# jenndrei/BayHunter

Hardware: AMD Instinct MI355X
Metric: forward-model+logL evals/sec (batched 10-layer models) (higher is better)
Workload: dtype f64

## Files before the change

### bayhunter_amd/csrc/bh_device.h

```cpp
#pragma once
#include <hip/hip_runtime.h>
#include <stddef.h>
#include <stdint.h>

#define BH_WAVE 64
#define BH_COUNTER_WORDS 16
#define BH_TRACE_WAVES 16384
#define BH_DEBUG_WORDS (BH_COUNTER_WORDS + 4 * BH_TRACE_WAVES)
#define BH_BOARD_WORDS (2 * 32768)

__device__ __forceinline__ double bh_rcp_refined(double b)
{
    double r = __builtin_amdgcn_rcp(b);
    double e = __builtin_fma(-b, r, 1.0);
    r = __builtin_fma(r, e, r);
    e = __builtin_fma(-b, r, 1.0);
    r = __builtin_fma(r, e, r);
    return r;
}
__device__ __forceinline__ double bh_quot(double a, double b, double r)
{
    const double q = a * r;
    const double rem = __builtin_fma(-b, q, a);
    return __builtin_fma(rem, r, q);
// ... 72 lines not shown
    int Lcut;
    int rows[2], lanes[2];
    int wg_n0, wg_n1;
    unsigned long long *neval;
    unsigned *board;
    unsigned stamp;
    unsigned *started;
    int prio_low;
    int fast;
    int adapt_ok;
    int counted;
    int rerun;
    int farith;
    int restart;
    SwdTarget t[8];
};
struct SwdSiteXArgs {
    const int32_t *site;
    int nsites, nt, ldx;
    const int32_t *n;
    const double *x;
    int col[8], off[8];
};
__device__ __forceinline__ int bh_site_count(const SwdSiteXArgs &X, int ty, int ib, int cap)
{
    const int s = X.site[ib];
    if (s < 0 || s >= X.nsites) return -1;
    const int n = X.n[(size_t)s * X.nt + X.col[ty]];
    return n < 0 ? 0 : (n > cap ? cap : n);
}
// ... 8 lines not shown
double bh_swd_plan(int B, int Lmax, int ntargets, const int *iwave, int Gforce, int *G, int *look);
size_t bh_swd_group_lds_bytes(int G, int J, int Lmax, int Kmax, int maxmode, bool sitex = false);
struct SwdPairWork {
    int ncu = 0;
    int32_t *perm[2] = {nullptr, nullptr};
    int32_t *slot_rank[2] = {nullptr, nullptr};
    int cap_perm = 0, cap_rank[2] = {0, 0};
    int key_n0 = -1, key_n1 = -1;
};
struct PairOrderTarget {
    int mpw, nwaves;
    const int32_t *slot_rank;
    int32_t *perm;
    int xcd;
};
bool bh_pair_order_fits(int B);
void bh_launch_pair_order(int B, int Lmax, const int32_t *nlay, const double *vs, ptrdiff_t sl, ptrdiff_t sb, int nt,
                          const PairOrderTarget *tg, hipStream_t stream);
struct SwdLaunchInfo {
    unsigned workgroups;
    long waves;
    size_t lds;
    int wpb;
};
inline int bh_trials_fit(int G, int look)
{
    int J = look > 1 ? look : 1;
    while (J > 1 && G * J > BH_WAVE) --J;
    return J;
}
struct SwdGroupAsk {
// ... 174 lines not shown
```

### bayhunter_amd/csrc/bh_engine.hip

```cpp
#include "../../include/bh_engine_debug.h"
#include "../../include/bh_engine_sites.h"
#include "../../include/bh_engine_sites_rf.h"
#include "../../include/bh_engine_sites_x.h"
#include "../../include/bh_engine_sites_x_all.h"
#include "../../include/bh_engine_sites_missing.h"
#include "../../include/bh_engine_sites_gauss.h"
#include "../../include/bh_engine_sites_rf_axis.h"
#include "bh_device.h"

#include <algorithm>
#include <cmath>
#include <cstdio>
#include <cstdlib>
#include <cstring>
#include <new>
#include <string>
#include <vector>

#include "bh_tuning.h"
#include <cstring>
#include <mutex>

namespace {
BhTuning g_tuning;
// ... 121 lines not shown
    DevBuf gc_xn;
    DevBuf gc_work;
    bool timing = false, counting = false;
    bool no_mfma = false;
    bool as_given = false;
    int force_group = 0;
    int force_look = 0;
    int hint_layers = 0;
    int swd_search = BH_SEARCH_FAST;
    int swd_arith = BH_ARITH_FAST;
    int swd_scan = 2;
    DevBuf guard;
    uint64_t rerun_launches = 0;
    uint64_t guard_total[BH_MAX_TARGETS] = {0};
    bool guard_fresh = true;
    bool guard_last = false;
    struct EventSet {
        hipEvent_t ev[8];
        bool used[4];
    };
    std::vector<EventSet> evsets;
    size_t ncalls = 0;
    uint64_t last_neval = 0;
    bool neval_pending = false;
};

namespace {

int fail(bh_engine *e, int code, const char *what, hipError_t he = hipSuccess)
{
// ... 195 lines not shown
int swd_counter(bh_engine *e, hipStream_t st, unsigned long long **out)
{
    *out = nullptr;
    if (!e->counting) return BH_OK;
    int rc = ensure(e, e->counter, BH_DEBUG_WORDS * sizeof(unsigned long long));
    if (rc) return rc;
    if (!e->neval_pending) {
        HIPCHK(e, hipMemsetAsync(e->counter.p, 0, BH_COUNTER_WORDS * sizeof(unsigned long long), st));
        e->neval_pending = true;
    }
    *out = (unsigned long long *)e->counter.p;
    return BH_OK;
}

constexpr int GUARD_HEAD = 24;
int guard_space(bh_engine *e, hipStream_t st, int B, int32_t **counts, int32_t **lists)
{
    const size_t need = ((size_t)GUARD_HEAD + (size_t)BH_MAX_TARGETS * (size_t)(B + 4)) * sizeof(int32_t);
    if (need > e->guard.cap) {
        if (e->guard.p) {
            int32_t cum[BH_MAX_TARGETS];
            HIPCHK(e, hipStreamSynchronize(st));
            HIPCHK(e, hipMemcpy(cum, (int32_t *)e->guard.p + 2 * BH_MAX_TARGETS, sizeof(cum), hipMemcpyDeviceToHost));
            for (int t = 0; t < BH_MAX_TARGETS; ++t) e->guard_total[t] += (uint64_t)(uint32_t)cum[t];
        }
        e->guard_fresh = true;
    }
    int rc = ensure(e, e->guard, need);
    if (rc) return rc;
    *counts = (int32_t *)e->guard.p;
    *lists = (int32_t *)e->guard.p + GUARD_HEAD;
    HIPCHK(e, hipMemsetAsync(e->guard.p, 0, (e->guard_fresh ? GUARD_HEAD : 2 * BH_MAX_TARGETS) * sizeof(int32_t), st));
    e->guard_fresh = false;
    return BH_OK;
}

bool takes_fast(int search, const SwdJob &J)
{
    return J.igr == BH_VEL_PHASE && J.mode <= 1 && (search == BH_SEARCH_FAST || (search == BH_SEARCH_FAST_RAYLEIGH && J.iwave == BH_WAVE_RAYLEIGH));
}

enum SwdOrder { ORDER_NONE, ORDER_DEPTH, ORDER_LENGTH, ORDER_PAIR };

struct SwdPlan {
    bool first_roots[BH_MAX_TARGETS];
    int nsplit;
    int ntargets, kmax, maxmode;
    bool any_sphere;
    int typ_layers;
    int kernel;
    int G, lean_trials;
    int order, Lcut;
    int len_mpw, len_xcd;
    bool sitex;
    bool any_fast, farith, adapt_ok;
    int job[BH_MAX_TARGETS], look[BH_MAX_TARGETS], inlook[BH_MAX_TARGETS], look_group[BH_MAX_TARGETS];
    bool fast[BH_MAX_TARGETS], refseq[BH_MAX_TARGETS];
};

SwdPlan plan_swd(const bh_engine *e, int B, int Lmax, int typ_given, int njobs, const SwdJob *jobs)
{
    const BhTuning &tun = bh_tuning();
    SwdPlan p{};
    p.maxmode = 1;
    for (int j = 0; j < njobs; ++j) p.sitex = p.sitex || jobs[j].sx.tab != nullptr;
    int iw[BH_MAX_TARGETS], nfast = 0;
    for (int j = 0; j < njobs; ++j) {
        const SwdJob &J = jobs[j];
// ... 45 lines not shown
            wmax = w > wmax ? w : wmax;
        }
        const int pair_min = tun.swd_pair_minwaves;
        if (plan_waves >= (pair_min >= 0 ? pair_min : 7 * (long)e->pairwork.ncu) && (pair_min >= 0 || 2 * wmax >= 3 * wmin))
            p.order = ORDER_PAIR;
    }
    p.Lcut = Lmax;
    if (ordered && p.order != ORDER_PAIR) {
        if (lean && bh_pair_order_fits(B) && tun.swd_lean_no_sort == 0) {
            p.order = ORDER_LENGTH;
            p.len_mpw = 1;
            const int mpw = BH_WAVE / p.lean_trials, per_wg = (nlive == 2) ? 2 : 4;
            if (tun.swd_lean_xcd != 0 && tun.swd_lean_r < 4 && tun.swd_lean_l < 4 && B % mpw == 0 && B % 8 == 0 && (B / mpw) % (8 * per_wg) == 0) {
                p.len_mpw = mpw;
                p.len_xcd = per_wg;
            }
        } else {
            p.order = ORDER_DEPTH;
            if (shallow_bulk) p.Lcut = p.typ_layers + 2;
        }
    }
    p.any_fast = nfast > 0;
    p.farith = e->swd_arith == BH_ARITH_FAST;
    p.adapt_ok = e->force_group == 0 && e->force_look == 0 && tun.swd_look_r == 0 && tun.swd_look_l == 0;
    for (int t = 0; t < nlive; ++t) {
        p.refseq[t] = nfast > 0 && jobs[p.job[t]].igr == BH_VEL_PHASE && !p.fast[t];
        if (p.kernel == BH_KERNEL_LANE) {
            p.look[t] = look[t] > 1 ? look[t] : 1;
            continue;
        }
// ... 168 lines not shown
}

unsigned swd_stamp(bh_engine *e)
{
    const unsigned s = (++e->swd_stamp) & 0xffffu;
    return s != 0 ? s : (++e->swd_stamp) & 0xffffu;
}

int wait_for(bh_engine *e, hipEvent_t ev, hipStream_t from, hipStream_t to)
{
    HIPCHK(e, hipEventRecord(ev, from));
    HIPCHK(e, hipStreamWaitEvent(to, ev, 0));
    return BH_OK;
}

void note_launch(bh_engine *e, int family, int role, const int key[6], bool two, bool inter, bool pair, bool restart, unsigned grid_x, int fair)
{
    if (e->n_swd_launches >= (int)(sizeof(e->swd_launches) / sizeof(e->swd_launches[0]))) return;
    bh_swd_launch &r = e->swd_launches[e->n_swd_launches++];
    r.family = family; r.role = role;
    for (int k = 0; k < 6; ++k) r.key[k] = key[k];
    r.two_classes = two; r.interleaved = inter; r.pair_order = pair; r.restart = restart; r.grid_x = (int)grid_x; r.fair = fair;
}
void note_lane(bh_engine *e, int role, const SwdLaneBuild &b) { note_launch(e, BH_KERNEL_LANE, role, b.key, false, false, false, false, b.grid_x, b.fair); }
void note_group(bh_engine *e, int role, const SwdGroupPlan &g, bool pair)
{
    const SwdGroupBuild &b = g.build;
    const int key[6] = {b.fastm, b.simple, b.prof, b.adapt, b.cntb, b.fa};
    note_launch(e, BH_KERNEL_GROUP, role, key, g.grid.z == 2, g.wg_n1 > 0, pair, g.restart, g.grid.x, 0);
}

void set_group_args(SwdMultiArgs &a, const SwdGroupPlan &g)
{
    for (int k = 0; k < 2; ++k) {
        a.rows[k] = g.rows[k];
        a.lanes[k] = g.lanes[k];
    }
// ... 52 lines not shown
            target_of(W, ty, wid);
            if (ty == t && wid < nw[t] - 1) v.emplace_back(q[(size_t)W], wid);
        }
        std::sort(v.begin(), v.end());
        rank[t].assign((size_t)(nw[t] > 0 ? nw[t] : 1), 0);
        for (size_t r = 0; r < v.size(); ++r) rank[t][(size_t)v[r].second] = (int32_t)r;
    }
    return true;
}

int launch_swd_rerun(bh_engine *e, hipStream_t st, const SwdMultiArgs &main, int32_t *counts, int32_t *lists, const SwdSiteXArgs *sx = nullptr)
{
    SwdMultiArgs a = main;
    a.rerun = 1;
    a.perm = nullptr;
    a.split = nullptr;
    a.Lcut = a.Lmax;
    a.started = nullptr;
    a.stamp = swd_stamp(e);
    a.adapt_ok = 1;
    SwdGroupAsk q{};
    q.B = a.B; q.Lmax = q.Lcut = a.Lmax; q.ntargets = a.ntargets;
    q.G0 = bh_swd_pick_group(a.B, a.ntargets, a.Lmax);
    for (int t = 0; t < a.ntargets; ++t) {
        SwdTarget &T = a.t[t];
        T.perm = lists + (size_t)t * (size_t)(a.B + 4);
        T.count = counts + t;
        T.gcount = nullptr;
        T.glist = nullptr;
        T.look = 64 / q.G0 > 1 ? 64 / q.G0 : 1;
// ... 50 lines not shown
        PairOrderTarget tg[2];
        for (int t = 0; t < nt; ++t) tg[t] = PairOrderTarget{g.pair_mpw[t], n[t], geom ? pw.slot_rank[t] : nullptr, pw.perm[t]};
        const SwdTarget t0 = swd_target(c, c.p.job[0]);
        bh_launch_pair_order(B, c.Lmax, c.m.nlay, t0.vs, t0.sl, t0.sb, nt, tg, c.st);
        for (int t = 0; t < nt; ++t) c.pair_perm[t] = pw.perm[t];
    }
    (void)hipGetLastError();
    return BH_OK;
}

int order_models(SwdCall &c)
{
    const SwdPlan &p = c.p;
    if (p.order == ORDER_NONE) return BH_OK;
    if (p.order == ORDER_PAIR) return c.g.pair ? pair_models(c) : BH_OK;
    bh_engine *e = c.e;
    int rc;
    if ((rc = ensure(e, e->perm, ((size_t)c.B + 4) * sizeof(int32_t)))) return rc;
    int32_t *perm = (int32_t *)e->perm.p;
    if (p.order == ORDER_LENGTH) {
        const PairOrderTarget tg{p.len_mpw, c.B / p.len_mpw, nullptr, perm + 4, p.len_xcd};
        bh_launch_pair_order(c.B, c.Lmax, c.m.nlay, c.m.vs, c.sl, c.sb, 1, &tg, c.st);
    } else {
        bh_launch_order(c.B, c.m.nlay, perm + 4, p.Lcut, perm, c.st);
        c.split = (p.Lcut < c.Lmax) ? perm : nullptr;
    }
    c.perm = perm + 4;
    return BH_OK;
}

// ... 35 lines not shown
    if (fork && (rc = wait_for(e, e->ev_join2, e->aux2, c.st))) return rc;
    HIPCHK(e, hipGetLastError());
    return BH_OK;
}

int launch_swd_multi(SwdCall &c, SwdMultiArgs &a)
{
    bh_engine *e = c.e;
    const SwdPlan &p = c.p;
    const int B = c.B;
    int rc;
    if ((rc = swd_board(e, c.st, &a.board))) return rc;
    a.stamp = swd_stamp(e);
    a.B = B; a.Lmax = c.Lmax; a.nlay = c.m.nlay; a.neval = c.counter; a.perm = c.perm;
    a.split = c.split; a.Lcut = p.Lcut;
    a.ntargets = p.ntargets;
    for (int t = 0; t < p.ntargets; ++t) {
        a.t[t] = swd_target(c, p.job[t]);
        a.t[t].look = p.look[t];
        a.t[t].inlook = p.inlook[t];
        a.t[t].refseq = p.refseq[t] ? 1 : 0;
    }
    a.started = e->started;
    a.prio_low = c.prio_low;
    a.adapt_ok = p.adapt_ok ? 1 : 0;
    if (p.sitex) {
        c.sx = *c.jobs[p.job[0]].sx.tab;
        for (int t = 0; t < p.ntargets; ++t) {
            c.sx.col[t] = c.jobs[p.job[t]].sx.col;
            c.sx.off[t] = c.jobs[p.job[t]].sx.off;
// ... 5 lines not shown
        a.farith = p.farith ? 1 : 0;
        a.fast = p.any_fast ? 1 : 0;
    } else {
        for (int t = 0; t < 2; ++t) a.t[t].perm = c.pair_perm[t];
        set_group_args(a, c.g);
    }
    if (bh_tuning().debug_plan != 0) {
        std::fprintf(stderr, "[bh] dispersion plan B=%d Lmax=%d: lanes per model %d, typical layers %d (hint %d), Lcut %d%s, pairing %d; trials per round:",
                     B, c.Lmax, p.G, c.m.typ_layers, e->hint_layers, p.Lcut, p.Lcut < c.Lmax ? " (two depth classes)" : "", (int)(p.order == ORDER_PAIR));
        for (int t = 0; t < p.ntargets; ++t) std::fprintf(stderr, " %s %d/%d", a.t[t].iwave == BH_WAVE_LOVE ? "L" : "R", p.look_group[t], p.inlook[t]);
        if (!lean) std::fprintf(stderr, "; launched lanes per model %d/%d", c.g.lanes[0], c.g.lanes[1]);
        std::fprintf(stderr, "\n");
    }
    e->guard_last = p.any_fast;
    if (p.any_fast) {
        if ((rc = guard_space(e, c.st, B, &c.gcounts, &c.glists))) return rc;
        for (int t = 0; t < a.ntargets; ++t)
            if (a.t[t].igr == BH_VEL_PHASE) {
                a.t[t].gcount = c.gcounts + t;
                a.t[t].glist = c.glists + (size_t)t * (size_t)(B + 4);
            }
    }
    ev_begin(e, 0, c.st);
    e->last_swd_kernel = p.kernel;
    if (lean) {
        SwdLaneBuild lb{};
        if ((p.sitex ? bh_launch_swd_lean_x(a, c.sx, c.st, &c.info, &lb) : bh_launch_swd_lean(a, c.st, &c.info, &lb)) != 0)
            return fail(e, BH_EINVAL, "model too deep for LDS");
        note_launch(e, BH_KERNEL_LEAN, BH_SWD_MAIN, lb.key, false, p.ntargets == 2, false, false, lb.grid_x, 0);
    } else {
        if (!p.sitex) bh_launch_swd_group(a, c.g, c.st);
        else if (!bh_launch_swd_group_x(a, c.g, c.sx, c.st)) return fail(e, BH_EUNSUPPORTED, "no site-period build of this dispersion launch");
        note_group(e, BH_SWD_MAIN, c.g, c.pair_perm[0] != nullptr);
        c.info = c.g.info;
    }
    const hipError_t le = hipGetLastError();
    if (le != hipSuccess) return fail(e, BH_EHIP, "dispersion kernel launch", le);
    if (e->started) e->started_expected += c.info.workgroups;
    return BH_OK;
}

int launch_second_roots(const SwdCall &c)
{
    bh_engine *e = c.e;
    const int B = c.B;
    const bool sitex = c.p.sitex && e->site_x_all;
    int J2 = 16;
    {
        long searches = 0;
        for (int t = 0; t < c.p.ntargets; ++t) searches += c.p.first_roots[c.p.job[t]] ? (long)B * c.jobs[c.p.job[t]].K : 0;
        while (J2 > 1 && searches * J2 > 2048L * 64) J2 >>= 1;
    }
    size_t off[BH_MAX_TARGETS + 1] = {0};
// ... 273 lines not shown
}
int bh_engine_set_swd_trials(bh_engine *e, int trials)
{
    if (!e) return BH_EINVAL;
    if (trials != 0 && trials != 4 && trials != 8 && trials != 16 && trials != 32 && trials != 64)
        return fail(e, BH_EINVAL, "trials must be 0 (by the call's shape), 4, 8, 16, 32 or 64");
    e->swd_trials = trials;
    return BH_OK;
}
int bh_engine_get_swd_trials(const bh_engine *e) { return e ? e->swd_trials : 0; }
int bh_engine_guard_stats(bh_engine *e, int32_t *counts, uint64_t *rerun_launches, uint64_t *total)
{
    if (!e) return BH_EINVAL;
    if (rerun_launches) *rerun_launches = e->rerun_launches;
    if (counts || total) {
        int32_t w[3 * BH_MAX_TARGETS] = {0};
        if (e->guard.p && !e->guard_fresh) {
            HIPCHK(e, hipDeviceSynchronize());
            HIPCHK(e, hipMemcpy(w, e->guard.p, sizeof(w), hipMemcpyDeviceToHost));
        }
        if (counts)
            for (int t = 0; t < BH_MAX_TARGETS; ++t) counts[t] = e->guard_last ? w[t] + w[BH_MAX_TARGETS + t] : 0;
        if (total)
            for (int t = 0; t < BH_MAX_TARGETS; ++t) total[t] = e->guard_total[t] + (uint64_t)(uint32_t)w[2 * BH_MAX_TARGETS + t];
    }
    return BH_OK;
}

int bh_engine_set_swd_lookahead(bh_engine *e, int trials_per_round)
{
    if (!e) return BH_EINVAL;
    if (trials_per_round < 0 || trials_per_round > 16)
        return fail(e, BH_EINVAL, "look-ahead must be 0 (auto) or 1..16 trial velocities per round");
    e->force_look = trials_per_round;
    return BH_OK;
}

int bh_engine_set_swd_group(bh_engine *e, int lanes_per_model)
{
// ... 861 lines not shown
```

### bayhunter_amd/csrc/bh_tuning.h

```cpp
#pragma once

#define BH_TUNING_TABLE(X)                                                                                                          \
    X(swd_search,        "BH_SWD_SEARCH",        -1, "initial root refinement: r(eference) / f(ast) / fast_rayleigh; -1 = the library's default")    \
    X(swd_scan,          "BH_SWD_SCAN",          -1, "initial scan mode: s(teps) / c(ounted) / a(uto); -1 = auto")                                  \
    X(swd_arith,         "BH_SWD_ARITH",         -1, "initial arithmetic of short-refinement launches: e(xact) / f(ast); -1 = the library's default") \
    X(swd_group,         "BH_SWD_GROUP",          0, "lanes per model of the dispersion kernel (0 = planned per launch)")                           \
    X(swd_lookahead,     "BH_SWD_LOOKAHEAD",      0, "trial velocities per round (0 = planned per launch)")                                         \
    X(swd_look_r,        "BH_SWD_LOOK_R",         0, "trials per round of Rayleigh wavefronts only (0 = planned)")                                  \
    X(swd_look_l,        "BH_SWD_LOOK_L",         0, "trials per round of Love wavefronts only (0 = planned)")                                      \
    X(swd_love_inlook,   "BH_SWD_LOVE_INLOOK",    0, "Love trials inside a lane group, 1..4 (0 = automatic)")                                       \
    X(swd_prio_low,      "BH_SWD_PRIO_LOW",      -1, "issue priority of a dispersion wavefront's unfavoured phase beside RF wavefronts (-1 = 1)")    \
    X(swd_pair_minwaves, "BH_SWD_PAIR_MINWAVES", -1, "wavefronts from which the SIMD-pairing order of the models is used (-1 = 7 x CUs)")           \
    X(swd_slice,         "BH_SWD_SLICE",          0, "lane-per-model kernel: rounds between priority changes (0 = default)")                        \
    X(swd_hint_always,   "BH_SWD_HINT_ALWAYS",    0, "flag: honour the typical-depth hint also when every model gets a wavefront")                   \
    X(swd_no_pair,       "BH_SWD_NO_PAIR",        0, "flag: no SIMD-pairing order of the models")                                                    \
    X(swd_no_mix,        "BH_SWD_NO_MIX",         0, "flag: Rayleigh and Love wavefronts not interleaved in the grid")                               \
    X(swd_no_adapt,      "BH_SWD_NO_ADAPT",       0, "flag: one-model-per-wavefront launches do not size lane groups per model")                     \
    X(swd_no_restart,    "BH_SWD_NO_RESTART",     0, "flag: guarded models are re-run by a second launch instead of restarting in place")            \
    X(swd_no_simple,     "BH_SWD_NO_SIMPLE",      0, "flag: no kernel build specialised for fundamental-mode phase velocities")                      \
    X(swd_no_board,      "BH_SWD_NO_BOARD",       0, "flag: no progress board between the two wavefronts of a SIMD")                                 \
    X(swd_no_fair,       "BH_SWD_NO_FAIR",        0, "flag: no alternating issue priority of the two wavefronts of a SIMD")                          \
    X(swd_redundant,     "BH_SWD_REDUNDANT",      0, "flag: every lane of a group runs the whole Rayleigh recursion")                                \
    X(swd_no_lean,       "BH_SWD_NO_LEAN",        0, "flag: fast-arithmetic launches take the group / lane kernels' FA builds, not the trial-per-lane kernel") \
    X(swd_lean_pairs,    "BH_SWD_LEAN_PAIRS",     0, "trial-per-lane kernel: largest call in (model, target) pairs that takes it (0 = 2^20)")        \
    X(swd_lean_no_sort,  "BH_SWD_LEAN_NO_SORT",   0, "flag: trial-per-lane kernel: models by depth only, not by predicted search length")           \
    X(swd_lean_r,        "BH_SWD_LEAN_R",         0, "trial-per-lane kernel: trials per round of Rayleigh targets, power of two 4..64 (0 = planned)")  \
    X(swd_lean_l,        "BH_SWD_LEAN_L",         0, "trial-per-lane kernel: trials per round of Love targets (0 = planned)")                         \
    X(swd_lean_xcd,      "BH_SWD_LEAN_XCD",       1, "trial-per-lane kernel: 1 = the models ordered inside eight blocks of the batch, a block per XCD (0: one order for the chip)") \
    X(swd_rerun_wgs,     "BH_SWD_RERUN_WGS",    256, "workgroups per target of the re-run launch of guarded models, striding over the list (0 = one wavefront per model of the batch, as before round 6)") \
    X(swd_gsplit,        "BH_SWD_GSPLIT",  16777216, "group velocities (fundamental mode): calls of up to this many (model, period) pairs per target -- 2^24, the most the launch indexes -- run the chain of first roots and the second roots as two launches (0 = one search after the other in one launch)") \
    X(swd_lean_flip,     "BH_SWD_LEAN_FLIP",    256, "trial-per-lane kernel, two targets: 256 = the second target takes the models in the opposite order (0: the same order); + n: the targets of a wavefront pair swap with bit n-1 of the workgroup index") \
    X(no_order,          "BH_NO_ORDER",           0, "flag: models processed in the caller's order")                                                 \
    X(no_overlap,        "BH_NO_OVERLAP",         0, "flag: receiver function after the dispersion kernel, not beside it")                           \
    X(no_started,        "BH_NO_STARTED",         0, "flag: no start gate (stream memory operation) for the receiver-function stream")               \
    X(no_mfma,           "BH_NO_MFMA",            0, "flag: Gauss-law quadratic form in like_kernel instead of the MFMA contraction")                \
    X(err_memset,        "BH_ERR_MEMSET",         0, "flag: zero the per-target failure flags on every call")                                        \
    X(gauss_tile,        "BH_GAUSS_TILE",         0, "tile of the Gauss-law contraction: 64 / 128 (0 = automatic)")                                  \
    X(rf_lds_beside,     "BH_RF_LDS_BESIDE",     -1, "LDS floor (bytes) of receiver-function workgroups beside an ungated dispersion launch (-1 = default)") \
    X(rf_lds_gated,      "BH_RF_LDS_GATED",       0, "LDS floor (bytes) of receiver-function workgroups of a gated fused call (0 = none)")           \
    X(rf_keep_floor,     "BH_RF_KEEP_FLOOR",      0, "flag: keep the ungated LDS floor in a gated fused call")                                       \
    X(rf_coef_big,       "BH_RF_COEF_BIG",        0, "flag: the large-register coefficient kernel also beside the dispersion kernel")                \
    X(rf_no_fuse,        "BH_RF_NO_FUSE",         0, "flag: the receiver function always writes its trace (no fused likelihood)")                    \
    X(rf_no_cut,         "BH_RF_NO_CUT",          0, "flag: every frequency bin computed (no spectral cut-off below 1e-17)")                         \
// ... 17 lines not shown
```

### bayhunter_amd/csrc/swd_kernel.hip

```cpp
#include "../../include/bh_engine_debug.h"
#include "bh_device.h"
#include "bh_tuning.h"
#include <cmath>
#include <cstdlib>

#define BH_HD __device__ __forceinline__
#define BH_TAB static __device__ const
#include "bh_libm.h"

namespace {
#include "swd_common.h"

constexpr int LANE_TAB_PAD = (LIBM_TAB_BYTES + 15) & ~15;
#ifndef BH_NEV_LO
#define BH_NEV_LO 5
#endif
constexpr int NEV_LO = BH_NEV_LO;
__host__ __device__ inline size_t lane_wave_bytes(int Lmax, int K, int mode)
{
    const size_t b = (size_t)4 * Lmax * 64 * sizeof(float) + (size_t)2 * NEV_LO * 64 * sizeof(double) +
                     (size_t)((K + 1) & ~1) * sizeof(double) + (mode > 1 ? (size_t)2 * K * 64 * sizeof(double) : 0);
    return (b + 15) & ~(size_t)15;
}

// ... 295 lines not shown
        __syncthreads();
        bin[tid] = (wv > 0 ? wsum[wv - 1] : 0) + acc - mine;
        __syncthreads();
    }
#pragma unroll
    for (int i = 0; i < PER_THREAD; ++i)
        if (tid + 1024 * i < B) sorted[atomicAdd(&bin[bucket(i)], 1)] = tid + 1024 * i;
    __syncthreads();
    for (int t = 0; t < nt; ++t) {
        const PairOrderTarget T = t == 0 ? t0 : t1;
        for (int pos = tid; pos < B; pos += 1024) {
            const int wid = pos / T.mpw, m = pos - wid * T.mpw;
            int src = pos;
            if (!ragged && T.slot_rank != nullptr && wid < T.nwaves - 1) src = T.slot_rank[wid] * T.mpw + m;
            if (blocked) {
                const int x = (T.xcd == 2) ? (wid >> 1) & 7 : (wid >> 2) & 7;
                const int q = (T.xcd == 2) ? (((wid >> 4) << 1) | (wid & 1)) : (((wid >> 5) << 2) | (wid & 3));
                src = x * per + q * T.mpw + m;
            }
            T.perm[pos] = sorted[src];
        }
    }
}

__device__ __forceinline__ double sphere_log(double x)
{
    double y;
    return bhp_log(x, &y, bhp_log_data) ? y : log(x);
}
__device__ __forceinline__ float sphere_powf(float x, float y)
{
    float r;
// ... 273 lines not shown
```

### bayhunter_amd/csrc/swd_lean.hip

```cpp
#include "../../include/bh_engine_debug.h"
#include "bh_device.h"
#include "bh_tuning.h"
#include <algorithm>
#define BH_HD __device__ __forceinline__
#define BH_TAB static __device__ const
#include "bh_libm.h"
#ifndef BH_SWD_SITEX
#define BH_SWD_SITEX 0
#endif

namespace {
#include "swd_common.h"

struct LeanModel {
    const double *p;
    int S, LS;
    __device__ __forceinline__ double D(int m) const { return p[m * S]; }
    __device__ __forceinline__ double A(int m) const { return p[LS + m * S]; }
    __device__ __forceinline__ double Bv(int m) const { return p[2 * LS + m * S]; }
    __device__ __forceinline__ double R(int m) const { return p[3 * LS + m * S]; }
    __device__ __forceinline__ double IA(int m) const { return p[4 * LS + m * S]; }
    __device__ __forceinline__ double IB(int m) const { return p[5 * LS + m * S]; }
    __device__ __forceinline__ double IR(int m) const { return p[6 * LS + m * S]; }
};
// ... 73 lines not shown

#ifndef BH_LEAN_CLUSTER_W
#define BH_LEAN_CLUSTER_W 4.0e-7
#endif
#ifndef BH_LEAN_RIDE_TOL
#define BH_LEAN_RIDE_TOL 4.0e-7
#endif
#ifndef BH_LEAN_CLUSTER_BIG
#define BH_LEAN_CLUSTER_BIG 8
#endif
#ifndef BH_LEAN_CLUSTER
#define BH_LEAN_CLUSTER 2
#endif
constexpr int LEAN_WPB = 4;

template <int J, bool CNT>
#if BH_SWD_SITEX
__global__ __launch_bounds__(BH_WAVE * LEAN_WPB) void swd_lean_kernel(SwdMultiArgs A, int wave_lds, int flip, SwdSiteXArgs X)
#else
__global__ __launch_bounds__(BH_WAVE * LEAN_WPB) void swd_lean_kernel(SwdMultiArgs A, int wave_lds, int flip)
#endif
{
    if (A.started != nullptr && threadIdx.x == 0) atomicAdd(A.started, 1u);
    const int lane = threadIdx.x & (BH_WAVE - 1);
    const int wave = __builtin_amdgcn_readfirstlane((int)(threadIdx.x / BH_WAVE));
    int wid = (int)blockIdx.x * LEAN_WPB + wave, ty = (int)blockIdx.y;
    if (A.wg_n1 > 0) {
        const long long n1 = A.wg_n1, N = (long long)A.wg_n0 + n1;
        if (wid >= (int)N) return;
        const int l0 = (int)(((long long)wid * n1) / N), l1 = (int)((((long long)wid + 1) * n1) / N);
        ty = (l1 > l0) ? 1 : 0;
        wid = (l1 > l0) ? l0 : wid - l0;
        if ((flip & 256) && ty == 1) {
            if (flip & 2048) {
                const int x = (wid >> 1) & 7, q = ((wid >> 4) << 1) | (wid & 1), qr = A.wg_n1 / 8 - 1 - q;
                wid = ((qr >> 1) << 4) + 2 * x + (qr & 1);
            } else {
                wid = A.wg_n1 - 1 - wid;
            }
        }
    }
    const SwdTarget T = A.t[ty];
    constexpr int MPW = BH_WAVE / J;
    if (wid * MPW >= A.B) return;
    const int g = lane / J, r = lane & (J - 1), lbase = lane & ~(J - 1);
    const int sidx = wid * MPW + g;
    const bool valid = sidx < A.B;
    const int32_t *perm = T.perm != nullptr ? T.perm : A.perm;
    const int ib = valid ? (perm ? perm[sidx] : sidx) : 0;
    extern __shared__ __align__(16) unsigned char smem_lean[];
    constexpr double dc = (double)0.005f, onea = (double)1.5f, twopi = 2.0 * 3.141592653589793, guard_rel = 3.0e-6;
#if BH_SWD_SITEX
    const int Lmax = A.Lmax, Kcap = T.K, ifunc = T.iwave, KE = (Kcap + 1) & ~1;
    const int Kown = valid ? bh_site_count(X, ty, ib, Kcap) : 0;
    const int K = Kown > 0 ? Kown : 0;
    double *omg_all = reinterpret_cast<double *>(smem_lean + (size_t)wave * wave_lds);
    double *mdl = omg_all + MPW * KE;
    const double *omg = omg_all + g * KE;
    const int LS = Lmax * MPW;
    for (int idx = lane; idx < MPW * Kcap; idx += BH_WAVE) {
        const int mg = idx / Kcap, kk = idx - mg * Kcap;
        const int sbx = wid * MPW + mg;
        if (sbx < A.B) {
            const double *pr = X.x;
            const int kb = bh_site_periods(X, ty, perm ? perm[sbx] : sbx, Kcap, pr);
            if (kk < kb) omg_all[mg * KE + kk] = twopi / pr[kk];
        }
    }
#else
    const int Lmax = A.Lmax, K = T.K, ifunc = T.iwave;
    double *omg = reinterpret_cast<double *>(smem_lean + (size_t)wave * wave_lds);
    double *mdl = omg + ((K + 1) & ~1);
    const int LS = Lmax * MPW;
    for (int k = lane; k < K; k += BH_WAVE) omg[k] = twopi / T.periods[k];
#endif
    for (int idx = lane; idx < LS; idx += BH_WAVE) {
        const int l = idx / MPW, mg = idx - l * MPW;
        const int sb = wid * MPW + mg;
        const int b = sb < A.B ? (perm ? perm[sb] : sb) : 0;
        float fd = 0.f, fa_ = 1.f, fb = 1.f, fr = 1.f;
        if (sb < A.B && l < A.nlay[b]) {
            const ptrdiff_t o = (ptrdiff_t)b * T.sb + (ptrdiff_t)l * T.sl;
            fd = (float)T.h[o];
            fa_ = (float)T.vp[o];
            fb = (float)T.vs[o];
            fr = (float)T.rho[o];
        }
        mdl[idx] = (double)fd;
        mdl[LS + idx] = (double)fa_;
        mdl[2 * LS + idx] = (double)fb;
        mdl[3 * LS + idx] = (double)fr;
        mdl[4 * LS + idx] = fa::rcp((double)fa_);
        mdl[5 * LS + idx] = fa::rcp((double)fb);
        mdl[6 * LS + idx] = fa::rcp((double)fr);
// ... 577 lines not shown
{
    SwdMultiArgs a = a0;
    int kmax = 0, jmin = BH_WAVE;
    long wmax = 1, wsum = 0, nw[BH_MAX_TARGETS] = {0};
    for (int t = 0; t < a.ntargets; ++t) {
        const int J = a.t[t].look;
        if (J < 4 || J > BH_WAVE || (J & (J - 1)) != 0 || a.t[t].igr != 0 || a.t[t].mode > 1) return -1;
        kmax = a.t[t].K > kmax ? a.t[t].K : kmax;
        jmin = J < jmin ? J : jmin;
        const int mpw = BH_WAVE / J;
        nw[t] = (a.B + mpw - 1) / mpw;
        wmax = nw[t] > wmax ? nw[t] : wmax;
        wsum += nw[t];
    }
    const size_t wave_lds = lean_wave_lds(jmin, a.Lmax, kmax, BH_SWD_SITEX != 0);
    const size_t lds = LEAN_WPB * wave_lds;
    if (lds > 64 * 1024) return -1;
    dim3 grid((unsigned)((wmax + LEAN_WPB - 1) / LEAN_WPB), (unsigned)a.ntargets);
    a.wg_n0 = a.wg_n1 = 0;
    if (a.ntargets == 2) {
        a.wg_n0 = (int)nw[0];
        a.wg_n1 = (int)nw[1];
        grid = dim3((unsigned)((wsum + LEAN_WPB - 1) / LEAN_WPB), 1);
    }
    const dim3 block(BH_WAVE * LEAN_WPB);
    if (info != nullptr) {
        info->workgroups = grid.x * grid.y;
        info->waves = wsum;
        info->lds = lds;
        info->wpb = LEAN_WPB;
    }
    int flip = bh_tuning().swd_lean_flip;
// ... 30 lines not shown
```

### bayhunter_amd/engine.py

```python
import contextlib
import ctypes as C
import os
import sys

import numpy as np

_HERE = os.path.dirname(os.path.abspath(__file__))
LIB_PATH = os.path.join(_HERE, "libbh_engine.so")

BH_OK, BH_EINVAL, BH_EHIP, BH_ENOMEM, BH_EUNSUPPORTED = 0, -1, -2, -3, -4
HOST, DEVICE = 0, 1
WAVE_LOVE, WAVE_RAYLEIGH = 1, 2
VEL_PHASE, VEL_GROUP = 0, 1
RF_P, RF_SV = 0, 1
LAW_NOCORR, LAW_NOCORR_SCALED, LAW_EXP, LAW_GAUSS = 0, 1, 2, 3
TARGET_SWD, TARGET_RF, TARGET_USER = 0, 1, 2
SEARCH_REFERENCE, SEARCH_FAST, SEARCH_FAST_RAYLEIGH = 0, 1, 2
ARITH_EXACT, ARITH_FAST = 0, 1
SCAN_STEPS, SCAN_COUNTED, SCAN_AUTO = 0, 1, 2
MAX_PERIODS, MAX_LAYERS, MAX_TARGETS = 60, 100, 8

_d = C.POINTER(C.c_double)
_i32 = C.POINTER(C.c_int32)


class EngineError(RuntimeError):
    pass


class SwdLaunch(C.Structure):
    _fields_ = [("family", C.c_int), ("role", C.c_int), ("key", C.c_int * 6), ("two_classes", C.c_int), ("interleaved", C.c_int),
                ("pair_order", C.c_int), ("restart", C.c_int), ("grid_x", C.c_int), ("fair", C.c_int)]


class TargetDesc(C.Structure):
    _fields_ = [("kind", C.c_int32), ("law", C.c_int32), ("n", C.c_int32),
                ("iwave", C.c_int32), ("igr", C.c_int32), ("mode", C.c_int32), ("flsph", C.c_int32),
                ("waveno", C.c_int32), ("nsamp", C.c_int32),
                ("p_s_per_deg", C.c_double), ("gauss", C.c_double), ("fsamp", C.c_double),
                ("tshift", C.c_double), ("nsv", C.c_double),
                ("x", _d), ("yobs", _d), ("yerr", _d), ("rinv", _d), ("logdet_r", C.c_double)]


BH_MAX_TARGETS = 8
BH_CHAIN_MAXLAYERS = 32
BH_CHAIN_MAXDEPTH = 7

# ... 269 lines not shown
        try:
            yield self
        finally:
            if trials is not None:
                self.set_swd_trials(prev)

    def last_swd_kernel(self):
        return {0: "group", 1: "lane", 2: "lean"}.get(self._L.bh_engine_last_swd_kernel(self._h))

    def last_swd_launches(self):
        out = (SwdLaunch * 32)()
        n = C.c_int(0)
        self._check(self._L.bh_engine_last_swd_launches(self._h, out, 32, C.byref(n)))
        return [dict(family={0: "group", 1: "lane", 2: "lean"}[r.family], role={0: "main", 1: "rerun", 2: "second"}[r.role],
                     key=tuple(r.key), two_classes=bool(r.two_classes), interleaved=bool(r.interleaved),
                     pair_order=bool(r.pair_order), restart=bool(r.restart), grid_x=int(r.grid_x), fair=int(r.fair))
                for r in out[:n.value]]

    def swd_arith(self):
        return "fast" if self._L.bh_engine_get_swd_arith(self._h) == ARITH_FAST else "exact"

    @contextlib.contextmanager
    def computing(self, arith):
        prev = self.swd_arith()
        self.set_swd_arith(arith)
        try:
            yield self
        finally:
            self.set_swd_arith(prev)

    def set_swd_scan(self, scan):
# ... 332 lines not shown
```

### include/bh_engine_debug.h

```cpp
#ifndef BH_ENGINE_DEBUG_H
#define BH_ENGINE_DEBUG_H

#include "bh_engine.h"

#ifdef __cplusplus
extern "C" {
#endif

int bh_engine_set_swd_group(bh_engine *e, int lanes_per_model);
int bh_engine_set_swd_lookahead(bh_engine *e, int trials_per_round);

#define BH_KERNEL_GROUP 0
#define BH_KERNEL_LANE 1
#define BH_KERNEL_LEAN 2
int bh_engine_last_swd_kernel(const bh_engine *e);

typedef struct {
    int family, role, key[6];
    int two_classes, interleaved, pair_order, restart, grid_x, fair;
} bh_swd_launch;
#define BH_SWD_MAIN 0
#define BH_SWD_RERUN 1
#define BH_SWD_SECOND 2
int bh_engine_last_swd_launches(const bh_engine *e, bh_swd_launch *out, int max, int *n);

#define BH_SCAN_STEPS 0
#define BH_SCAN_COUNTED 1
#define BH_SCAN_AUTO 2
int bh_engine_set_swd_scan(bh_engine *e, int scan);
int bh_engine_get_swd_scan(const bh_engine *e);

int bh_engine_set_tuning(bh_engine *e, const char *name, int value);
int bh_engine_get_tuning(bh_engine *e, const char *name, int *value);

// ... 16 lines not shown
```

Measured before the change: 6.091 million.

## Compute per-XCD model order inside lean kernel prologue and self-zero guard heads

Instead of a separate ordering launch ahead of the lean dispersion kernel, each workgroup bucket-sorts its XCD block of models by velocity span or layer count in LDS during its prologue and picks its models from that order. The guard counters are double-buffered so the kernel zeroes the next head itself, which drops a per-call memset. Together these remove a kernel launch and a memset per call. In exchange every workgroup repeats the sort of its block, which adds prologue work and LDS use.

```diff
diff --git a/bayhunter_amd/csrc/bh_device.h b/bayhunter_amd/csrc/bh_device.h
--- a/bayhunter_amd/csrc/bh_device.h
+++ b/bayhunter_amd/csrc/bh_device.h
@@ -110,6 +110,8 @@
     int farith;
     int restart;
     SwdTarget t[8];
+    int order_in_kernel;
+    int32_t *zero_head;
 };
 struct SwdSiteXArgs {
     const int32_t *site;
@@ -148,7 +150,23 @@
     int32_t *perm;
     int xcd;
 };
+__host__ __device__ __forceinline__ void bh_lean_xcd_slot(int wid, int per_wg, int &x, int &q)
+{
+    x = (per_wg == 2) ? (wid >> 1) & 7 : (wid >> 2) & 7;
+    q = (per_wg == 2) ? (((wid >> 4) << 1) | (wid & 1)) : (((wid >> 5) << 2) | (wid & 3));
+}
+__host__ __device__ __forceinline__ int bh_lean_xcd_wid(int x, int q, int per_wg)
+{
+    return (per_wg == 2) ? ((q >> 1) << 4) + 2 * x + (q & 1) : ((q >> 2) << 5) + 4 * x + (q & 3);
+}
 bool bh_pair_order_fits(int B);
+constexpr int BH_LEAN_ORDER_BUCKETS = 128;
+constexpr size_t BH_LEAN_ORDER_MAX_LDS = 16 * 1024;
+inline size_t bh_swd_lean_order_bytes(int per)
+{
+    return (((size_t)per * 9 + 15) & ~(size_t)15) + (size_t)(3 * BH_LEAN_ORDER_BUCKETS + 16) * sizeof(int32_t);
+}
+inline bool bh_swd_lean_order_fits(int per) { return per >= 1 && per < 65536 && bh_swd_lean_order_bytes(per) <= BH_LEAN_ORDER_MAX_LDS; }
 void bh_launch_pair_order(int B, int Lmax, const int32_t *nlay, const double *vs, ptrdiff_t sl, ptrdiff_t sb, int nt,
                           const PairOrderTarget *tg, hipStream_t stream);
 struct SwdLaunchInfo {
diff --git a/bayhunter_amd/csrc/bh_engine.hip b/bayhunter_amd/csrc/bh_engine.hip
--- a/bayhunter_amd/csrc/bh_engine.hip
+++ b/bayhunter_amd/csrc/bh_engine.hip
@@ -159,6 +159,8 @@
     uint64_t rerun_launches = 0;
     uint64_t guard_total[BH_MAX_TARGETS] = {0};
     bool guard_fresh = true;
+    int guard_head = 0;
+    int guard_clean = -1;
     bool guard_last = false;
     struct EventSet {
         hipEvent_t ev[8];
@@ -384,24 +386,34 @@
 }
 
 constexpr int GUARD_HEAD = 24;
-int guard_space(bh_engine *e, hipStream_t st, int B, int32_t **counts, int32_t **lists)
-{
-    const size_t need = ((size_t)GUARD_HEAD + (size_t)BH_MAX_TARGETS * (size_t)(B + 4)) * sizeof(int32_t);
+int guard_space(bh_engine *e, hipStream_t st, int B, int32_t **counts, int32_t **lists, bool self_zeroing = false)
+{
+    const size_t need = ((size_t)2 * GUARD_HEAD + (size_t)BH_MAX_TARGETS * (size_t)(B + 4)) * sizeof(int32_t);
     if (need > e->guard.cap) {
         if (e->guard.p) {
-            int32_t cum[BH_MAX_TARGETS];
+            int32_t w[2 * GUARD_HEAD];
             HIPCHK(e, hipStreamSynchronize(st));
-            HIPCHK(e, hipMemcpy(cum, (int32_t *)e->guard.p + 2 * BH_MAX_TARGETS, sizeof(cum), hipMemcpyDeviceToHost));
-            for (int t = 0; t < BH_MAX_TARGETS; ++t) e->guard_total[t] += (uint64_t)(uint32_t)cum[t];
+            HIPCHK(e, hipMemcpy(w, e->guard.p, sizeof(w), hipMemcpyDeviceToHost));
+            for (int h = 0; h < 2; ++h)
+                for (int t = 0; t < BH_MAX_TARGETS; ++t) e->guard_total[t] += (uint64_t)(uint32_t)w[h * GUARD_HEAD + 2 * BH_MAX_TARGETS + t];
         }
         e->guard_fresh = true;
     }
     int rc = ensure(e, e->guard, need);
     if (rc) return rc;
-    *counts = (int32_t *)e->guard.p;
-    *lists = (int32_t *)e->guard.p + GUARD_HEAD;
-    HIPCHK(e, hipMemsetAsync(e->guard.p, 0, (e->guard_fresh ? GUARD_HEAD : 2 * BH_MAX_TARGETS) * sizeof(int32_t), st));
+    int head = 0;
+    if (e->guard_fresh) {
+        HIPCHK(e, hipMemsetAsync(e->guard.p, 0, 2 * GUARD_HEAD * sizeof(int32_t), st));
+    } else if (self_zeroing && e->guard_clean >= 0) {
+        head = e->guard_clean;
+    } else {
+        HIPCHK(e, hipMemsetAsync(e->guard.p, 0, 2 * BH_MAX_TARGETS * sizeof(int32_t), st));
+    }
     e->guard_fresh = false;
+    e->guard_head = head;
+    e->guard_clean = -1;
+    *counts = (int32_t *)e->guard.p + head * GUARD_HEAD;
+    *lists = (int32_t *)e->guard.p + 2 * GUARD_HEAD;
     return BH_OK;
 }
 
@@ -422,6 +434,7 @@
     int G, lean_trials;
     int order, Lcut;
     int len_mpw, len_xcd;
+    bool order_in_kernel;
     bool sitex;
     bool any_fast, farith, adapt_ok;
     int job[BH_MAX_TARGETS], look[BH_MAX_TARGETS], inlook[BH_MAX_TARGETS], look_group[BH_MAX_TARGETS];
@@ -497,6 +510,7 @@
             if (tun.swd_lean_xcd != 0 && tun.swd_lean_r < 4 && tun.swd_lean_l < 4 && B % mpw == 0 && B % 8 == 0 && (B / mpw) % (8 * per_wg) == 0) {
                 p.len_mpw = mpw;
                 p.len_xcd = per_wg;
+                p.order_in_kernel = tun.swd_lean_order_in_kernel != 0 && e->hint_layers == 0 && bh_swd_lean_order_fits(B / 8) && Lmax <= 255;
             }
         } else {
             p.order = ORDER_DEPTH;
@@ -695,13 +709,15 @@
     return BH_OK;
 }
 
-void note_launch(bh_engine *e, int family, int role, const int key[6], bool two, bool inter, bool pair, bool restart, unsigned grid_x, int fair)
+void note_launch(bh_engine *e, int family, int role, const int key[6], bool two, bool inter, bool pair, bool restart, unsigned grid_x, int fair,
+                 bool own_order = false)
 {
     if (e->n_swd_launches >= (int)(sizeof(e->swd_launches) / sizeof(e->swd_launches[0]))) return;
     bh_swd_launch &r = e->swd_launches[e->n_swd_launches++];
     r.family = family; r.role = role;
     for (int k = 0; k < 6; ++k) r.key[k] = key[k];
     r.two_classes = two; r.interleaved = inter; r.pair_order = pair; r.restart = restart; r.grid_x = (int)grid_x; r.fair = fair;
+    r.order_in_kernel = own_order;
 }
 void note_lane(bh_engine *e, int role, const SwdLaneBuild &b) { note_launch(e, BH_KERNEL_LANE, role, b.key, false, false, false, false, b.grid_x, b.fair); }
 void note_group(bh_engine *e, int role, const SwdGroupPlan &g, bool pair)
@@ -784,6 +800,8 @@
     SwdMultiArgs a = main;
     a.rerun = 1;
     a.perm = nullptr;
+    a.order_in_kernel = 0;
+    a.zero_head = nullptr;
     a.split = nullptr;
     a.Lcut = a.Lmax;
     a.started = nullptr;
@@ -864,6 +882,7 @@
     const SwdPlan &p = c.p;
     if (p.order == ORDER_NONE) return BH_OK;
     if (p.order == ORDER_PAIR) return c.g.pair ? pair_models(c) : BH_OK;
+    if (p.order_in_kernel) return BH_OK;
     bh_engine *e = c.e;
     int rc;
     if ((rc = ensure(e, e->perm, ((size_t)c.B + 4) * sizeof(int32_t)))) return rc;
@@ -929,6 +948,7 @@
     a.stamp = swd_stamp(e);
     a.B = B; a.Lmax = c.Lmax; a.nlay = c.m.nlay; a.neval = c.counter; a.perm = c.perm;
     a.split = c.split; a.Lcut = p.Lcut;
+    a.order_in_kernel = (p.kernel == BH_KERNEL_LEAN && p.order_in_kernel) ? 1 : 0;
     a.ntargets = p.ntargets;
     for (int t = 0; t < p.ntargets; ++t) {
         a.t[t] = swd_target(c, p.job[t]);
@@ -964,7 +984,8 @@
     }
     e->guard_last = p.any_fast;
     if (p.any_fast) {
-        if ((rc = guard_space(e, c.st, B, &c.gcounts, &c.glists))) return rc;
+        if ((rc = guard_space(e, c.st, B, &c.gcounts, &c.glists, lean))) return rc;
+        if (lean) a.zero_head = (int32_t *)e->guard.p + (1 - e->guard_head) * GUARD_HEAD;
         for (int t = 0; t < a.ntargets; ++t)
             if (a.t[t].igr == BH_VEL_PHASE) {
                 a.t[t].gcount = c.gcounts + t;
@@ -977,7 +998,7 @@
         SwdLaneBuild lb{};
         if ((p.sitex ? bh_launch_swd_lean_x(a, c.sx, c.st, &c.info, &lb) : bh_launch_swd_lean(a, c.st, &c.info, &lb)) != 0)
             return fail(e, BH_EINVAL, "model too deep for LDS");
-        note_launch(e, BH_KERNEL_LEAN, BH_SWD_MAIN, lb.key, false, p.ntargets == 2, false, false, lb.grid_x, 0);
+        note_launch(e, BH_KERNEL_LEAN, BH_SWD_MAIN, lb.key, false, p.ntargets == 2, false, false, lb.grid_x, 0, a.order_in_kernel != 0);
     } else {
         if (!p.sitex) bh_launch_swd_group(a, c.g, c.st);
         else if (!bh_launch_swd_group_x(a, c.g, c.sx, c.st)) return fail(e, BH_EUNSUPPORTED, "no site-period build of this dispersion launch");
@@ -987,6 +1008,7 @@
     const hipError_t le = hipGetLastError();
     if (le != hipSuccess) return fail(e, BH_EHIP, "dispersion kernel launch", le);
     if (e->started) e->started_expected += c.info.workgroups;
+    if (a.zero_head != nullptr) e->guard_clean = 1 - e->guard_head;
     return BH_OK;
 }
 
@@ -1290,15 +1312,16 @@
     if (!e) return BH_EINVAL;
     if (rerun_launches) *rerun_launches = e->rerun_launches;
     if (counts || total) {
-        int32_t w[3 * BH_MAX_TARGETS] = {0};
+        int32_t w2[2 * GUARD_HEAD] = {0};
+        const int32_t *w = w2 + e->guard_head * GUARD_HEAD, *wo = w2 + (1 - e->guard_head) * GUARD_HEAD;
         if (e->guard.p && !e->guard_fresh) {
             HIPCHK(e, hipDeviceSynchronize());
-            HIPCHK(e, hipMemcpy(w, e->guard.p, sizeof(w), hipMemcpyDeviceToHost));
+            HIPCHK(e, hipMemcpy(w2, e->guard.p, sizeof(w2), hipMemcpyDeviceToHost));
         }
         if (counts)
             for (int t = 0; t < BH_MAX_TARGETS; ++t) counts[t] = e->guard_last ? w[t] + w[BH_MAX_TARGETS + t] : 0;
         if (total)
-            for (int t = 0; t < BH_MAX_TARGETS; ++t) total[t] = e->guard_total[t] + (uint64_t)(uint32_t)w[2 * BH_MAX_TARGETS + t];
+            for (int t = 0; t < BH_MAX_TARGETS; ++t) total[t] = e->guard_total[t] + (uint64_t)(uint32_t)w[2 * BH_MAX_TARGETS + t] + (uint64_t)(uint32_t)wo[2 * BH_MAX_TARGETS + t];
     }
     return BH_OK;
 }
diff --git a/bayhunter_amd/csrc/bh_tuning.h b/bayhunter_amd/csrc/bh_tuning.h
--- a/bayhunter_amd/csrc/bh_tuning.h
+++ b/bayhunter_amd/csrc/bh_tuning.h
@@ -27,6 +27,7 @@
     X(swd_lean_r,        "BH_SWD_LEAN_R",         0, "trial-per-lane kernel: trials per round of Rayleigh targets, power of two 4..64 (0 = planned)")  \
     X(swd_lean_l,        "BH_SWD_LEAN_L",         0, "trial-per-lane kernel: trials per round of Love targets (0 = planned)")                         \
     X(swd_lean_xcd,      "BH_SWD_LEAN_XCD",       1, "trial-per-lane kernel: 1 = the models ordered inside eight blocks of the batch, a block per XCD (0: one order for the chip)") \
+    X(swd_lean_order_in_kernel, "BH_SWD_LEAN_ORDER_IN_KERNEL", 1, "trial-per-lane kernel: 1 = the per-XCD order of the models is computed by the kernel's workgroups in their prologue (0: by a launch of its own ahead of the kernel)") \
     X(swd_rerun_wgs,     "BH_SWD_RERUN_WGS",    256, "workgroups per target of the re-run launch of guarded models, striding over the list (0 = one wavefront per model of the batch, as before round 6)") \
     X(swd_gsplit,        "BH_SWD_GSPLIT",  16777216, "group velocities (fundamental mode): calls of up to this many (model, period) pairs per target -- 2^24, the most the launch indexes -- run the chain of first roots and the second roots as two launches (0 = one search after the other in one launch)") \
     X(swd_lean_flip,     "BH_SWD_LEAN_FLIP",    256, "trial-per-lane kernel, two targets: 256 = the second target takes the models in the opposite order (0: the same order); + n: the targets of a wavefront pair swap with bit n-1 of the workgroup index") \
diff --git a/bayhunter_amd/csrc/swd_kernel.hip b/bayhunter_amd/csrc/swd_kernel.hip
--- a/bayhunter_amd/csrc/swd_kernel.hip
+++ b/bayhunter_amd/csrc/swd_kernel.hip
@@ -333,8 +333,8 @@
             int src = pos;
             if (!ragged && T.slot_rank != nullptr && wid < T.nwaves - 1) src = T.slot_rank[wid] * T.mpw + m;
             if (blocked) {
-                const int x = (T.xcd == 2) ? (wid >> 1) & 7 : (wid >> 2) & 7;
-                const int q = (T.xcd == 2) ? (((wid >> 4) << 1) | (wid & 1)) : (((wid >> 5) << 2) | (wid & 3));
+                int x, q;
+                bh_lean_xcd_slot(wid, T.xcd, x, q);
                 src = x * per + q * T.mpw + m;
             }
             T.perm[pos] = sorted[src];
diff --git a/bayhunter_amd/csrc/swd_lean.hip b/bayhunter_amd/csrc/swd_lean.hip
--- a/bayhunter_amd/csrc/swd_lean.hip
+++ b/bayhunter_amd/csrc/swd_lean.hip
@@ -111,6 +111,118 @@
 #endif
 constexpr int LEAN_WPB = 4;
 
+template <int MPW>
+__device__ __forceinline__ int lean_block_order(const SwdMultiArgs &A, unsigned char *scr, int x, int q, int lane, int wave)
+{
+    constexpr int NB = BH_LEAN_ORDER_BUCKETS, NT = BH_WAVE * LEAN_WPB;
+    static_assert(NB == 2 * BH_WAVE, "the scan below gives every lane two buckets");
+    const int tid = threadIdx.x, per = A.B / 8, base = x * per;
+    int *cnt = reinterpret_cast<int *>(scr);
+    int *cur = cnt + NB;
+    int *start = cur + NB;
+    unsigned *red = reinterpret_cast<unsigned *>(start + NB);
+    float *cost = reinterpret_cast<float *>(red + 16);
+    unsigned short *la = reinterpret_cast<unsigned short *>(cost + per), *lb = la + per;
+    unsigned char *depth = reinterpret_cast<unsigned char *>(lb + per);
+    for (int i = tid; i < NB; i += NT) cnt[i] = 0;
+    unsigned tcmin = 0x7f800000u, tcmax = 0u, tnmin = 255u, tnmax = 0u;
+    auto keep = [&](int i, float lo, float hi, int n) {
+        float c = hi - lo;
+        c = (c >= 0.0f && c < 1e30f) ? c : 0.0f;
+        cost[i] = c;
+        depth[i] = (unsigned char)n;
+        const unsigned cb = __float_as_uint(c);
+        tcmin = cb < tcmin ? cb : tcmin;
+        tcmax = cb > tcmax ? cb : tcmax;
+        tnmin = (unsigned)n < tnmin ? (unsigned)n : tnmin;
+        tnmax = (unsigned)n > tnmax ? (unsigned)n : tnmax;
+    };
+    const double *vs = A.t[0].vs;
+    const ptrdiff_t sl = A.t[0].sl, sb = A.t[0].sb;
+    if (sb <= sl) {
+        for (int i = tid; i < per; i += NT) {
+            const int b = base + i;
+            int n = A.nlay[b];
+            n = n < 1 ? 1 : (n > A.Lmax ? A.Lmax : n);
+            float lo = 1e30f, hi = -1e30f;
+            for (int l = 0; l < n; ++l) {
+                const float v = (float)vs[(ptrdiff_t)b * sb + (ptrdiff_t)l * sl];
+                lo = v < lo ? v : lo;
+                hi = v > hi ? v : hi;
+            }
+            keep(i, lo, hi, n);
+        }
+    } else {
+        for (int i = tid >> 3; i < per; i += NT / 8) {
+            const int b = base + i;
+            int n = A.nlay[b];
+            n = n < 1 ? 1 : (n > A.Lmax ? A.Lmax : n);
+            float lo = 1e30f, hi = -1e30f;
+            for (int l = tid & 7; l < n; l += 8) {
+                const float v = (float)vs[(ptrdiff_t)b * sb + (ptrdiff_t)l * sl];
+                lo = v < lo ? v : lo;
+                hi = v > hi ? v : hi;
+            }
+            for (int off = 1; off < 8; off <<= 1) {
+                const float ol = __shfl_xor(lo, off), oh = __shfl_xor(hi, off);
+                lo = ol < lo ? ol : lo;
+                hi = oh > hi ? oh : hi;
+            }
+            if ((tid & 7) == 0) keep(i, lo, hi, n);
+        }
+    }
+    for (int off = 32; off > 0; off >>= 1) {
+        tcmin = min(tcmin, (unsigned)__shfl_xor((int)tcmin, off));
+        tcmax = max(tcmax, (unsigned)__shfl_xor((int)tcmax, off));
+        tnmin = min(tnmin, (unsigned)__shfl_xor((int)tnmin, off));
+        tnmax = max(tnmax, (unsigned)__shfl_xor((int)tnmax, off));
+    }
+    if (lane == 0) {
+        red[4 * wave] = tcmin;
+        red[4 * wave + 1] = tcmax;
+        red[4 * wave + 2] = tnmin;
+        red[4 * wave + 3] = tnmax;
+    }
+    __syncthreads();
+    for (int w = 0; w < LEAN_WPB; ++w) {
+        tcmin = min(tcmin, red[4 * w]);
+        tcmax = max(tcmax, red[4 * w + 1]);
+        tnmin = min(tnmin, red[4 * w + 2]);
+        tnmax = max(tnmax, red[4 * w + 3]);
+    }
+    const bool ragged = tnmin != tnmax;
+    const float cmin = __uint_as_float(tcmin), cmax = __uint_as_float(tcmax);
+    const float scale = (cmax > cmin) ? (float)(NB - 1) / (cmax - cmin) : 0.0f;
+    auto bucket = [&](int i) {
+        int k = ragged ? (int)tnmax - (int)depth[i] : (int)((cmax - cost[i]) * scale);
+        return k < 0 ? 0 : (k > NB - 1 ? NB - 1 : k);
+    };
+    for (int i = tid; i < per; i += NT) atomicAdd(&cnt[bucket(i)], 1);
+    __syncthreads();
+    if (wave == 0) {
+        const int c0 = cnt[2 * lane], c1 = cnt[2 * lane + 1];
+        int acc = c0 + c1;
+        for (int off = 1; off < BH_WAVE; off <<= 1) {
+            const int o = __shfl_up(acc, off);
+            if (lane >= off) acc += o;
+        }
+        acc -= c0 + c1;
+        start[2 * lane] = cur[2 * lane] = acc;
+        start[2 * lane + 1] = cur[2 * lane + 1] = acc + c0;
+    }
+    __syncthreads();
+    for (int i = tid; i < per; i += NT) la[atomicAdd(&cur[bucket(i)], 1)] = (unsigned short)i;
+    __syncthreads();
+    for (int p = tid; p < per; p += NT) {
+        const int i = la[p], k = bucket(i), s = start[k], e = s + cnt[k];
+        int rank = s;
+        for (int j = s; j < e; ++j) rank += (la[j] < i) ? 1 : 0;
+        lb[rank] = (unsigned short)i;
+    }
+    __syncthreads();
+    return base + (int)lb[q * MPW + (lane & (MPW - 1))];
+}
+
 template <int J, bool CNT>
 #if BH_SWD_SITEX
 __global__ __launch_bounds__(BH_WAVE * LEAN_WPB) void swd_lean_kernel(SwdMultiArgs A, int wave_lds, int flip, SwdSiteXArgs X)
@@ -130,8 +242,9 @@
         wid = (l1 > l0) ? l0 : wid - l0;
         if ((flip & 256) && ty == 1) {
             if (flip & 2048) {
-                const int x = (wid >> 1) & 7, q = ((wid >> 4) << 1) | (wid & 1), qr = A.wg_n1 / 8 - 1 - q;
-                wid = ((qr >> 1) << 4) + 2 * x + (qr & 1);
+                int x, q;
+                bh_lean_xcd_slot(wid, 2, x, q);
+                wid = bh_lean_xcd_wid(x, A.wg_n1 / 8 - 1 - q, 2);
             } else {
                 wid = A.wg_n1 - 1 - wid;
             }
@@ -144,8 +257,18 @@
     const int sidx = wid * MPW + g;
     const bool valid = sidx < A.B;
     const int32_t *perm = T.perm != nullptr ? T.perm : A.perm;
-    const int ib = valid ? (perm ? perm[sidx] : sidx) : 0;
     extern __shared__ __align__(16) unsigned char smem_lean[];
+    if (A.zero_head != nullptr && blockIdx.x == 0 && blockIdx.y == 0 && threadIdx.x < 2 * BH_MAX_TARGETS) A.zero_head[threadIdx.x] = 0;
+    const bool ink = A.order_in_kernel != 0;
+    int ibw = 0;
+    if (ink) {
+        int x, q;
+        bh_lean_xcd_slot(wid, A.wg_n1 > 0 ? 2 : LEAN_WPB, x, q);
+        ibw = lean_block_order<MPW>(A, smem_lean, x, q, lane, wave);
+        __syncthreads();
+    }
+    auto model_of = [&](int s_, int mg_) -> int { return ink ? __shfl(ibw, mg_) : (perm ? perm[s_] : s_); };
+    const int ib = valid ? model_of(sidx, g) : 0;
     constexpr double dc = (double)0.005f, onea = (double)1.5f, twopi = 2.0 * 3.141592653589793, guard_rel = 3.0e-6;
 #if BH_SWD_SITEX
     const int Lmax = A.Lmax, Kcap = T.K, ifunc = T.iwave, KE = (Kcap + 1) & ~1;
@@ -160,7 +283,7 @@
         const int sbx = wid * MPW + mg;
         if (sbx < A.B) {
             const double *pr = X.x;
-            const int kb = bh_site_periods(X, ty, perm ? perm[sbx] : sbx, Kcap, pr);
+            const int kb = bh_site_periods(X, ty, model_of(sbx, mg), Kcap, pr);
             if (kk < kb) omg_all[mg * KE + kk] = twopi / pr[kk];
         }
     }
@@ -174,7 +297,7 @@
     for (int idx = lane; idx < LS; idx += BH_WAVE) {
         const int l = idx / MPW, mg = idx - l * MPW;
         const int sb = wid * MPW + mg;
-        const int b = sb < A.B ? (perm ? perm[sb] : sb) : 0;
+        const int b = sb < A.B ? model_of(sb, mg) : 0;
         float fd = 0.f, fa_ = 1.f, fb = 1.f, fr = 1.f;
         if (sb < A.B && l < A.nlay[b]) {
             const ptrdiff_t o = (ptrdiff_t)b * T.sb + (ptrdiff_t)l * T.sl;
@@ -782,8 +905,15 @@
         wsum += nw[t];
     }
     const size_t wave_lds = lean_wave_lds(jmin, a.Lmax, kmax, BH_SWD_SITEX != 0);
-    const size_t lds = LEAN_WPB * wave_lds;
+    size_t lds = LEAN_WPB * wave_lds;
     if (lds > 64 * 1024) return -1;
+    if (a.order_in_kernel != 0) {
+        const int mpw = BH_WAVE / jmin, per_wg = a.ntargets == 2 ? 2 : LEAN_WPB;
+        bool ok = a.B % 8 == 0 && a.B % mpw == 0 && (a.B / mpw) % (8 * per_wg) == 0 && bh_swd_lean_order_fits(a.B / 8) && a.Lmax <= 255;
+        for (int t = 0; t < a.ntargets; ++t) ok = ok && a.t[t].look == jmin && a.t[t].perm == nullptr;
+        if (!ok || a.perm != nullptr) return -1;
+        lds = std::max(lds, bh_swd_lean_order_bytes(a.B / 8));
+    }
     dim3 grid((unsigned)((wmax + LEAN_WPB - 1) / LEAN_WPB), (unsigned)a.ntargets);
     a.wg_n0 = a.wg_n1 = 0;
     if (a.ntargets == 2) {
diff --git a/bayhunter_amd/engine.py b/bayhunter_amd/engine.py
--- a/bayhunter_amd/engine.py
+++ b/bayhunter_amd/engine.py
@@ -30,7 +30,8 @@
 
 class SwdLaunch(C.Structure):
     _fields_ = [("family", C.c_int), ("role", C.c_int), ("key", C.c_int * 6), ("two_classes", C.c_int), ("interleaved", C.c_int),
-                ("pair_order", C.c_int), ("restart", C.c_int), ("grid_x", C.c_int), ("fair", C.c_int)]
+                ("pair_order", C.c_int), ("restart", C.c_int), ("grid_x", C.c_int), ("fair", C.c_int),
+                ("order_in_kernel", C.c_int)]
 
 
 class TargetDesc(C.Structure):
@@ -330,7 +331,8 @@
         self._check(self._L.bh_engine_last_swd_launches(self._h, out, 32, C.byref(n)))
         return [dict(family={0: "group", 1: "lane", 2: "lean"}[r.family], role={0: "main", 1: "rerun", 2: "second"}[r.role],
                      key=tuple(r.key), two_classes=bool(r.two_classes), interleaved=bool(r.interleaved),
-                     pair_order=bool(r.pair_order), restart=bool(r.restart), grid_x=int(r.grid_x), fair=int(r.fair))
+                     pair_order=bool(r.pair_order), restart=bool(r.restart), grid_x=int(r.grid_x), fair=int(r.fair),
+                     order_in_kernel=bool(r.order_in_kernel))
                 for r in out[:n.value]]
 
     def swd_arith(self):
diff --git a/include/bh_engine_debug.h b/include/bh_engine_debug.h
--- a/include/bh_engine_debug.h
+++ b/include/bh_engine_debug.h
@@ -18,6 +18,7 @@
 typedef struct {
     int family, role, key[6];
     int two_classes, interleaved, pair_order, restart, grid_x, fair;
+    int order_in_kernel;
 } bh_swd_launch;
 #define BH_SWD_MAIN 0
 #define BH_SWD_RERUN 1
```

Result: no change. 6.050 million (-0.7%).
